# kokutoupan/burn_raymarching

Hardware: AMD Instinct MI355X
Metric: Mrays/s fwd+bwd, 512x512 / 256 spheres / 32 steps, at 1/2/4/8 MI355X (higher is better)
Workload: dtype f32

## Files before the change

burn_raymarching_amd/csrc/rm_kernels.hip:

```cpp
#include <hip/hip_runtime.h>
#include <hip/hip_ext.h>

#include <algorithm>
#include <cstdarg>
#include <cmath>
#include <cstdio>
#include <cstdlib>
#include <cstring>
#include <string>
#include <type_traits>
#include <utility>
#include <vector>

#include "../../include/raymarch.h"
#include "rm_device.h"

namespace rm {

constexpr int kOrderClasses = 16;
constexpr int kOrderClsStride = 32;
constexpr int kOrderCntStride = kOrderClasses * kOrderClsStride > 64 ? kOrderClasses * kOrderClsStride : 64;
static_assert(kOrderCntStride >= kOrderClasses * kOrderClsStride && kOrderCntStride % 32 == 0, "128-byte lines per set");
constexpr int kRedArrStride = 32;

// ... 688 lines not shown
    const int w = __builtin_amdgcn_readfirstlane(*a.oturn);
    const int r = (w + 2) % 3, z = (w + 1) % 3;
    constexpr long long kSet = (long long)kOrderClasses * kMaxBlocksPerLaunch;
    if (o.list_r != nullptr) {
      o.list_r += r * kSet;
      o.cnt_r += r * kOrderCntStride;
    }
    if (o.list_w != nullptr) {
      o.list_w += w * kSet;
      o.cnt_w += w * kOrderCntStride;
    }
    if (o.cnt_z != nullptr) o.cnt_z += z * kOrderCntStride;
  }
  return o;
}

__device__ __forceinline__ long long ray_block(const KArgs& a) {
  int b = blockIdx.x;
  if (a.block_order == nullptr) return b;
  const int g = b >> 3;
  if ((g + 1) * 8 <= (int)gridDim.x) b = (g << 3) + (((b & 7) + g) & 7);
  const OrderSets os = order_sets(a);
  if (os.cnt_r != nullptr) {
    int tot = 0, cb = -1, base = 0;
#pragma unroll
    for (int c = 0; c < kOrderClasses; ++c) {
      const int n = os.cnt_r[c * kOrderClsStride];
      if (cb < 0 && b < tot + n) {
        cb = c;
        base = tot;
      }
      tot += n;
    }
    if (tot == (int)gridDim.x && cb >= 0) return os.list_r[cb * kMaxBlocksPerLaunch + (b - base)];
  }
  const int r = b / a.order_views, v = b - r * a.order_views;
  return (long long)v * a.order_tiles + a.block_order[r];
}

__device__ __forceinline__ void order_append(const KArgs& a, long long blk, int cost) {
  constexpr int kCls = kOrderClasses;
  const float cls_scale = (float)kCls / (float)((a.split ? 1 : kWaves) * (a.steps + kPostCost) + 1);
  const int c = kCls - 1 - (int)fminf((float)cost * cls_scale, (float)(kCls - 1));
  const OrderSets os = order_sets(a);
  const int idx = atomicAdd(os.cnt_w + c * kOrderClsStride, 1);
  if (idx < kMaxBlocksPerLaunch) os.list_w[c * kMaxBlocksPerLaunch + idx] = (int)blk;
}

__device__ __forceinline__ float progress_of(const KArgs& a) {
  if (a.sdev == nullptr) return a.progress;
  return fminf((float)a.sdev->index / (float)a.sdev->total, 1.0f);
}

template <int MODE>
__device__ __forceinline__ void escaped_block(const KArgs& a, const Lds& L, long long blk, long long ri, bool valid,
                                           int tid, int lane, int wave) {
  if (MODE != kBwd && a.out != nullptr && valid) {
    a.out[3 * ri] = 0.0f;
    a.out[3 * ri + 1] = 0.0f;
    a.out[3 * ri + 2] = 0.0f;
  }
  if constexpr (MODE == kFwd || MODE == kRender) return;
  float* rec = a.partials + blk * a.rec;
  float loss = 0.0f;
  if (MODE == kTrain && valid) {
    const float t0 = a.targets[3 * ri], t1 = a.targets[3 * ri + 1], t2 = a.targets[3 * ri + 2];
    const float W = (t0 + t1 + t2) > 0.01f ? 10.0f : fmaf(progress_of(a), 4.0f, 1.0f);
    const float tg[3] = {t0, t1, t2};
#pragma unroll
    for (int c = 0; c < 3; ++c) loss = fmaf(fabsf(0.0f - tg[c]), W, loss);
  }
  const float vals[8] = {0.0f, 0.0f, 0.0f, 0.0f, loss, 0.0f, 0.0f, 0.0f};
  const float red = wave_reduce8(vals, lane);
  if ((lane & 7) == 7) L.slots[wave * 8 + (lane >> 3)] = red;
  __syncthreads();
  if (tid < 8) {
    float acc = L.slots[tid];
#pragma unroll
    for (int w = 1; w < kWaves; ++w) acc += L.slots[w * 8 + tid];
    rec[(long long)a.Mpad * 8 + tid] = acc;
  }
}

template <bool CAM>
__device__ __forceinline__ void setup_ray(const KArgs& a, long long& ri, float o[3], float d[3], int& view) {
  view = 0;
  if constexpr (CAM) {
    const long long npix = (long long)a.width * a.height;
    const int v = (int)(ri / npix);
    view = v;
    const long long pix = ri - (long long)v * npix;
    int x, y;
    if (a.tiling == 2) {
      const long long tl = pix >> 8;
      const int w = (int)(pix & 255), tiles_x = a.width >> 4;
      const int ty = (int)(tl / tiles_x), tx = (int)(tl - (long long)ty * tiles_x);
      const int qd = w >> 6, l = w & 63;
      y = (ty << 4) + ((qd >> 1) << 3) + (l >> 3);
      x = (tx << 4) + ((qd & 1) << 3) + (l & 7);
    } else {
      y = (int)(pix / a.width);
      x = (int)(pix - (long long)y * a.width);
    }
    ri = (long long)v * npix + (long long)y * a.width + x;
    if (a.cams_dev != nullptr) camera_ray(a.cams_dev[v], x, y, a.width, a.height, o, d);
    else camera_ray(a.cams[v], x, y, a.width, a.height, o, d);
  } else {
    o[0] = a.org[3 * ri];
    o[1] = a.org[3 * ri + 1];
    o[2] = a.org[3 * ri + 2];
    d[0] = a.dir[3 * ri];
    d[1] = a.dir[3 * ri + 1];
    d[2] = a.dir[3 * ri + 2];
  }
}

template <int MODE, bool CAM>
__global__ __launch_bounds__(kBlock) void rm_escape_kernel(const KArgs a, int* __restrict__ flags) {
  __shared__ float scratch[8 * kWaves];
  const int tid = threadIdx.x;
  const long long blk = ray_block(a);
  const long long li = blk * kBlock + tid;
  const bool valid = li < a.n_rays;
  long long ri = a.ray_begin + (valid ? li : 0);
  float o[3], d[3];
  int view;
  setup_ray<CAM>(a, ri, o, d, view);
  float c0[3], R;
  scene_bound(a, scratch, tid, c0, R);
  const bool have_t = MODE == kBwd && a.t_in != nullptr;
  const bool esc = !valid || escapes(o, d, have_t ? a.t_in[ri] : -1.0f, have_t, a.steps, c0, R, a.lse_slack,
                                     a.cull_min_d);
  const int all = __syncthreads_and(esc);
  if (tid == 0) flags[blk] = all;
}

#include "rm_ray.h"
#include "rm_reduce.h"
#include "rm_small.h"
#include "rm_raygrad.h"
#include "rm_view.h"
#include "rm_sdf.h"
#include "rm_sh.h"

__global__ __launch_bounds__(64) void rm_stall_kernel(const int* flag, unsigned long long max_ticks) {
  const unsigned long long t0 = __builtin_amdgcn_s_memrealtime();
  while (__hip_atomic_load(flag, __ATOMIC_RELAXED, __HIP_MEMORY_SCOPE_SYSTEM) == 0) {
    if (__builtin_amdgcn_s_memrealtime() - t0 > max_ticks) break;
    __builtin_amdgcn_s_sleep(100);
  }
}

}

#include "rm_context.h"
#include "rm_launch.h"
#include "rm_api.h"
```

burn_raymarching_amd/csrc/rm_proof.h:

```cpp
#pragma once

constexpr int kProofMinSpheres = 128;
constexpr int kLatticeN = 64;
constexpr float kLatticeMargin = 0.25f;
constexpr float kProofMinStep = 0.02f;

constexpr double kMarchAbs = 1e-3;
constexpr double kBoundStepAbs = 1e-3;
constexpr double kRadiusRel = 1e-6;
constexpr double kEscapeRel = 1e-5;
constexpr double kProofRel = 2e-5;
constexpr double kProofMaxMagnitude = 256.0;
constexpr double kLatticeHalfDiag = 0.8660254;
constexpr double kLatticeCellRel = 1e-4;
constexpr double kLatticeKernelAbs = 1e-3;
constexpr double kTileRootRel = 1e-6;
constexpr double kTileRootFloor = 1e-15;
constexpr double kTileLatticeRel = 2e-6;
constexpr double kTileRoundAbs = 1e-4;
constexpr double kTileConeRel = 1e-4;
constexpr double kTileConeAbs = 2e-6;
constexpr double kTileRecedeRel = 2e-6;
constexpr double kBallAbs = kMarchAbs + kBoundStepAbs;
constexpr double kTileLatticeAbs = kMarchAbs + kBoundStepAbs + kLatticeKernelAbs + kTileRoundAbs;
constexpr double kProofDistUp = 1.0000200005;
static_assert(kProofDistUp * (1.0 - kProofRel) >= 1.0 && kProofDistUp < 1.0 + 1.01 * kProofRel,
              "T kProofDistUp >= T / (1 - kProofRel), and no more than it has to be");
static_assert(kLatticeHalfDiag * (1.0 + kLatticeCellRel) > 0.86602540379 * (1.0 + 4e-5),
              "the slack's factor covers sqrt(3)/2 and the cell index's (1/2 + 2e-5) h per axis");
static_assert(kProofRel >= 2.0 * kEscapeRel && kTileLatticeAbs >= kBallAbs + kLatticeKernelAbs,
              "the bound point's test holds the march's own; the tile's lattice term charges what the cell's does");

__device__ __forceinline__ float proof_rprime(float R, float lse_slack) {
  return (R + lse_slack + (float)kMarchAbs) * (1.0f + (float)kRadiusRel);
}
```

burn_raymarching_amd/csrc/rm_ray.h:

```cpp
#pragma once

struct ContState {
  enum Row { kT = 0, kLb, kDprev, kCycT1, kCycT2, kCode, kRhoLb, kRhist, kRayRows };
  static constexpr int kGroupWords = 2;
  struct Ray {
    float t, lb, Dprev, cyc_t1, cyc_t2, rho_lb;
    int rhist;
    bool gone, retired;
  };
  float* cs;
  long long R;
  __host__ __device__ static size_t floats(long long rays, long long groups) {
    return (size_t)(kRayRows * rays + kGroupWords * groups);
  }
  __device__ __forceinline__ explicit ContState(const KArgs& a) : cs(a.cont_state), R(a.cont_rays) {}
  __device__ __forceinline__ float& row(int r, long long li) const { return cs[r * R + li]; }
  __device__ __forceinline__ float& group(long long blk, int w) const { return cs[kRayRows * R + kGroupWords * blk + w]; }
  __device__ __forceinline__ static float code(const Ray& s) { return s.gone ? 1.0f : (s.retired ? 2.0f : 0.0f); }
  __device__ __forceinline__ Ray load(long long li) const {
    Ray s;
    s.t = row(kT, li);
    s.lb = row(kLb, li);
    s.Dprev = row(kDprev, li);
    s.cyc_t1 = row(kCycT1, li);
// ... 49 lines not shown
      const float4 C3 = R4[lay.pair(RecLayout::kP3, i)];
      const float2 C4 = R2[i];
      s.rr = h ? R.w : R.z;
      s.cr = h ? C3.y : C3.x;
      s.cg = h ? C3.w : C3.z;
      s.cbl = h ? C4.y : C4.x;
    } else {
      s.kr = h ? R.y : R.x;
    }
  }
  return s;
}
__device__ __forceinline__ void add_cols4(float* rec, int j, const float (&v)[8]) {
  float4* dst = reinterpret_cast<float4*>(rec + (long long)j * 8);
  float4 o = dst[0];
  o.x += v[0];
  o.y += v[1];
  o.z += v[2];
  o.w += v[3];
  dst[0] = o;
}

template <int MODE, bool CAM, bool SPLIT, bool PROOF>
__device__ __forceinline__ void ray_body(const KArgs& a);

template <int MODE, bool CAM, bool SPLIT, bool PROOF>
__device__ __forceinline__ void ray_entry(const KArgs& a) {
#ifdef RM_BLOCK_TRACE
  const unsigned long long t_begin = __builtin_amdgcn_s_memrealtime();
  ray_body<MODE, CAM, SPLIT, PROOF>(a);
  const unsigned long long t_end = __builtin_amdgcn_s_memrealtime();
  if (a.btrace != nullptr && (threadIdx.x & 63) == 0) {
    const unsigned hw = __builtin_amdgcn_s_getreg((31 << 11) | 4);
    const unsigned xcc = __builtin_amdgcn_s_getreg((31 << 11) | 20);
    unsigned long long* r = a.btrace + kTraceWords * ((unsigned long long)blockIdx.x * kWaves + (threadIdx.x >> 6));
    r[0] = t_begin;
    r[1] = t_end;
    r[2] = (unsigned long long)hw | ((unsigned long long)xcc << 32);
    r[3] = (unsigned long long)ray_block(a) | ((unsigned long long)blockIdx.x << 32);
  }
#else
  ray_body<MODE, CAM, SPLIT, PROOF>(a);
#endif
}
template <int MODE, bool CAM, bool SPLIT, bool PROOF = false>
__global__ __launch_bounds__(kBlock, SPLIT ? kSplitMinWaves : kMinWavesPerSimd) void rm_ray_kernel(const KArgs a) {
  static_assert(!PROOF || (!SPLIT && MODE != kRender), "the escape proof: unsplit training kernels");
  ray_entry<MODE, CAM, SPLIT, PROOF>(a);
}

template <int MODE, bool CAM, bool SPLIT, bool PROOF>
__device__ __forceinline__ void ray_body(const KArgs& a) {
  extern __shared__ __attribute__((aligned(16))) unsigned char smem[];
  const Lds L = bind_lds(a, smem);

  const int tid = threadIdx.x, lane = tid & 63, wave = __builtin_amdgcn_readfirstlane(tid >> 6);
  long long blk;
  long long li_listed = -1;
  bool listed = true;
  if (SPLIT && a.cont_resume > 0 && a.ray_cont) {
    const int n = *a.ray_count;
    const int i0 = (int)blockIdx.x * kSplitRays;
    if (i0 >= n) return;
    const int i = i0 + (lane & (kSplitRays - 1));
    listed = i < n;
    li_listed = a.ray_list[listed ? i : i0];
    blk = -1;
  } else if (SPLIT && a.cont_resume > 0) {
    if ((int)blockIdx.x >= *a.cont_count) return;
    blk = a.cont_list[blockIdx.x];
  } else {
    blk = ray_block(a);
  }
  const long long li = li_listed >= 0 ? li_listed
                                      : (SPLIT ? blk * kSplitRays + (lane & (kSplitRays - 1)) : blk * kBlock + tid);
  const bool valid = listed && li < a.n_rays;
  long long ri = a.ray_begin + (valid ? li : 0);
  const bool own_rays = !SPLIT || (wave == 0 && lane < kSplitRays);

  const float kappa = a.k * kLog2e, nkappa = -kappa, inv_kappa = 1.0f / kappa;

  float o[3], d[3];
  int view;
  setup_ray<CAM>(a, ri, o, d, view);

  if (a.ocnt_z != nullptr && blockIdx.x == 0 && tid < kOrderClasses) order_sets(a).cnt_z[tid * kOrderClsStride] = 0;
  if (a.esc_flags != nullptr && blk >= 0 && a.esc_flags[blk]) {
    if (a.stats != nullptr && tid == 0) atomicAdd(a.stats, 1ull);
    if (a.ocnt_w != nullptr && tid == 0) order_append(a, blk, 0);
    escaped_block<MODE>(a, L, blk, ri, valid, tid, lane, wave);
    return;
  }

  const cf1_ptr hdr = rec_header(L, a.Mpad);
  const float rmin = hdr[Hdr::kRmin], rmax = hdr[Hdr::kRmax], spread = hdr[Hdr::kSpread];
  const bool shift_fixed_ok = !a.shift_max && kappa * (rmax + spread) * 1.001f <= 100.0f;
  const bool shift_none_ok = !a.shift_max && kappa * rmax * 1.001f <= 30.0f;
  const float kr_first = kappa * a.radius[0];
  bool gone = false;
  bool retired = false;
  float rho_lb = -INFINITY;
  const float onorm = fabsf(o[0]) + fabsf(o[1]) + fabsf(o[2]);
  auto rho_moved = [&](float rl, float t0, float t1) {
    return rl - (fabsf(t1 - t0) * 1.000001f + 1e-6f * (1.0f + onorm + fmaxf(t0, t1)));
  };
  auto all_safe = [&](float dist_lb, float rlb) {
    return __all(dist_lb + rmin >= kSafeRho || rlb >= kSafeRho || gone) != 0;
  };
  int split_par = 0;

  auto soft_min = [&](const float p[3], bool fast, float& m, float& s) {
    m = -INFINITY;
    s = 0.0f;
    if (fast)
      lse_point<false, kShiftMax>(p, L, a.Mpad / 2, nkappa, m, s);
    else
      lse_point<true, kShiftMax>(p, L, a.Mpad / 2, nkappa, m, s);
    return -(flog2(fmaxf(s, 1e-8f)) + m) * inv_kappa;
  };
  auto split_pair = [&](int w) { return (((a.Mpad / 2) * w) / kSplitWaves) & ~7; };
  auto soft_min_split = [&](const float p[3], bool fast, float& m, float& s) {
    const int b0 = split_pair(wave), b1 = split_pair(wave + 1);
    const Lds Lq = L.from_pair(b0);
    m = -INFINITY;
    s = 0.0f;
    if (fast) lse_point<false, kShiftMax>(p, Lq, b1 - b0, nkappa, m, s);
    else lse_point<true, kShiftMax>(p, Lq, b1 - b0, nkappa, m, s);
    float* xm = L.slots;
    float* xs = L.slots + kSplitWaves * 64;
    __syncthreads();
    xm[wave * 64 + lane] = m;
    xs[wave * 64 + lane] = s;
    __syncthreads();
    float mm = xm[lane];
#pragma unroll
    for (int w = 1; w < kSplitWaves; ++w) mm = fmaxf(mm, xm[w * 64 + lane]);
    float ss = 0.0f;
#pragma unroll
    for (int w = 0; w < kSplitWaves; ++w) ss += xs[w * 64 + lane] * fexp2(xm[w * 64 + lane] - mm);
    m = mm;
    s = ss;
    return -(flog2(fmaxf(s, 1e-8f)) + m) * inv_kappa;
  };
  auto shade_merge = [&](float c10l, float& dmin, f2& Zw, f2 (&C)[3], f2& Zb, f2 (&G)[3]) {
    constexpr int kF = 9;
    float* xb = L.slots + 2 * kSplitWaves * 64;
    const float v[kF] = {dmin, Zw.x + Zw.y, C[0].x + C[0].y, C[1].x + C[1].y, C[2].x + C[2].y,
                         Zb.x + Zb.y, G[0].x + G[0].y, G[1].x + G[1].y, G[2].x + G[2].y};
#pragma unroll
    for (int f = 0; f < kF; ++f) xb[(f * kSplitWaves + wave) * 64 + lane] = v[f];
    __syncthreads();
    float dm = xb[lane];
#pragma unroll
    for (int w = 1; w < kSplitWaves; ++w) dm = fminf(dm, xb[w * 64 + lane]);
    float acc[kF - 1] = {0.0f, 0.0f, 0.0f, 0.0f, 0.0f, 0.0f, 0.0f, 0.0f};
#pragma unroll
    for (int w = 0; w < kSplitWaves; ++w) {
      const float dw = xb[w * 64 + lane];
      const float sw = fexp2((dm - dw) * c10l), sb = fexp2((dm - dw) * kappa);
#pragma unroll
      for (int f = 1; f < kF; ++f) acc[f - 1] = fmaf(xb[(f * kSplitWaves + w) * 64 + lane], f < 5 ? sw : sb, acc[f - 1]);
    }
    dmin = dm;
    Zw = f2{acc[0], 0.0f};
    C[0] = f2{acc[1], 0.0f};
    C[1] = f2{acc[2], 0.0f};
    C[2] = f2{acc[3], 0.0f};
    Zb = f2{acc[4], 0.0f};
    G[0] = f2{acc[5], 0.0f};
    G[1] = f2{acc[6], 0.0f};
    G[2] = f2{acc[7], 0.0f};
  };
#ifdef RM_BLOCK_TRACE
  unsigned long long tr_paths = 0, tr_lse_cyc = 0, tr_vec = 0;
// ... 155 lines not shown
          lat_inv_h = lg[Lat::kInvH];
          lat_slack = lg[Lat::kSlack] + (float)kBallAbs;
        }
      }
      float u = t;
      bool proven = gone || !valid;
      for (int n = st; n < a.steps; ++n) {
        const float ex = fmaf(d[0], u, o[0]) - c0x, ey = fmaf(d[1], u, o[1]) - c0y, ez = fmaf(d[2], u, o[2]) - c0z;
        const float dist = fsqrt(fmaf(ez, ez, fmaf(ey, ey, ex * ex)));
        const float Tn = esc_tab[min(a.steps - n, kEscTab - 1)];
        proven = proven || (fmaf(ez, d[2], fmaf(ey, d[1], ex * d[0])) >= 0.0f && dist * (1.0f - (float)kProofRel) >= Tn);
        if (__all(proven)) {
          steps_saved += a.steps - st;
          return true;
        }
        float Lb = dist - rs;
        if constexpr (CAM) {
          if (lat) {
            constexpr float kN = (float)kLatticeN;
            const int ix = (int)__builtin_floorf(__builtin_amdgcn_fmed3f((ex + lat_half) * lat_inv_h, -1.0f, kN));
            const int iy = (int)__builtin_floorf(__builtin_amdgcn_fmed3f((ey + lat_half) * lat_inv_h, -1.0f, kN));
            const int iz = (int)__builtin_floorf(__builtin_amdgcn_fmed3f((ez + lat_half) * lat_inv_h, -1.0f, kN));
            const bool inside = (unsigned)(ix | iy | iz) < (unsigned)kLatticeN;
            const int cx = min(max(ix, 0), kLatticeN - 1), cy = min(max(iy, 0), kLatticeN - 1),
                      cz = min(max(iz, 0), kLatticeN - 1);
            const float g = a.lattice[(cz * kLatticeN + cy) * kLatticeN + cx];
            Lb = fmaxf(Lb, inside ? g - lat_slack : -INFINITY);
          }
        }
        if (__any(!proven && !(Lb > kProofMinStep))) return false;
        u += proven ? 0.0f : Lb;
      }
      return false;
    };
    int st_stop = -1;
    int st0 = 0;
#ifdef RM_BLOCK_TRACE
    const unsigned long long tr_c_begin = __builtin_readcyclecounter();
    unsigned long long tr_cyc = 0;
#endif
    if constexpr (CAM) {
      if (a.origin != nullptr && a.steps > 0 && !(SPLIT && a.cont_resume > 0)) {
        const float D0 = a.origin[RecTail::kD0 + view];
        rho_lb = a.origin[RecTail::kRhoLb + view];
        if (__all((__float_as_uint(D0) & 0x7fffffffu) <= 0x7f800000u)) {
          const float p[3] = {fmaf(d[0], t, o[0]), fmaf(d[1], t, o[1]), fmaf(d[2], t, o[2])};
          if (wave_escaped(0, p)) {
            dead = true;
          } else {
            t = fminf(t + (gone ? gone_step : D0), kTMax);
            rho_lb = rho_moved(rho_lb, 0.0f, t);
            lb = D0 - fabsf(D0);
            Dprev = D0;
            st0 = 1;
            steps_saved = 1;
          }
        }
      }
    }
    float cyc_t1 = __builtin_nanf(""), cyc_t2 = __builtin_nanf("");
    int chist = 0xFFF;
    float Dprev2 = INFINITY;
    int rhist = 0xFFF;
    if (SPLIT && a.cont_resume > 0) {
      const ContState cs(a);
      const ContState::Ray s = cs.load(li);
      t = s.t;
      lb = s.lb;
      Dprev = s.Dprev;
      cyc_t1 = s.cyc_t1;
      cyc_t2 = s.cyc_t2;
      gone = s.gone;
      retired = s.retired;
      rho_lb = s.rho_lb;
      rhist = s.rhist;
      if (!a.ray_cont) {
        chist = __float_as_int(cs.group(blk, 0));
        steps_saved = __float_as_int(cs.group(blk, 1));
      }
      st0 = a.cont_resume;
    }
    if constexpr (PROOF) {
      bool taken = false;
      if constexpr (CAM) {
        if (!dead && a.tile_proof != nullptr) taken = a.tile_proof[blk * kWaves + wave] != 0;
      }
      if (taken) {
        steps_saved += a.steps - st0;
        dead = true;
      } else if (!dead && bound_proof(st0)) {
        dead = true;
      }
    }
    const unsigned long long below = (1ull << lane) - 1ull;
    for (int st = st0; !dead && st < a.steps; ++st) {
      if (SPLIT && a.cont_cap > 0 && st == a.cont_cap) {
        const ContState cs(a);
        const bool act = valid && !gone && !retired && lane < kSplitRays;
        gone_finish(st);
        if (wave == 0 && lane < kSplitRays && valid)
          cs.save(li, ContState::Ray{t, lb, Dprev, cyc_t1, cyc_t2, rho_lb, rhist, gone, retired});
        if (wave == 0) {
          const unsigned long long am = __ballot(act);
          const int na = __popcll(am);
          int base = 0;
          if (lane == 0 && na > 0) base = atomicAdd(a.ray_count_w, na);
          base = __shfl(base, 0);
          if (act) a.ray_list_w[base + __popcll(am & below)] = (int)li;
          if (lane == 0) {
            if (!a.ray_cont) {
              cs.group(blk, 0) = __int_as_float(chist);
              cs.group(blk, 1) = __int_as_float(steps_saved + (a.steps - st));
              a.cont_list_w[atomicAdd(a.cont_count_w, 1)] = (int)blk;
            } else if (a.stats != nullptr && st > st0) {
              atomicAdd(a.stats + 2, (unsigned long long)(-(long long)(st - st0)));
            }
          }
        }
        return;
      }
      const float p[3] = {fmaf(d[0], t, o[0]), fmaf(d[1], t, o[1]), fmaf(d[2], t, o[2])};
      if (wave_escaped(st, p)) {
        dead = true;
        st_stop = st;
        break;
      }
      int choice;
      const Memo mm{t, cyc_t1, cyc_t2, Dprev2, chist};
      const float D = soft_min_march(p, all_safe(lb, rho_lb), Dprev, choice, mm);
      const float t_step = t;
      if constexpr (SPLIT) {
        const float rl0 = rho_lb;
        if (!retired) {
          t = fminf(t + (gone ? gone_step : D), kTMax);
          rho_lb = rho_moved(rl0, t_step, t);
          lb = D - fabsf(D);
          Dprev = D;
        }
        if (a.early_exit && MODE != kRender) {
          if (!retired && !gone && valid && t_step == cyc_t2 && (choice & 3) == ((rhist >> 3) & 3)) {
            retired = true;
            if (((a.steps - st) & 1) == 0) {
              t = t_step;
              rho_lb = rl0;
            }
          }
          if (!retired) {
            cyc_t2 = cyc_t1;
            cyc_t1 = t_step;
          }
          rhist = ((rhist << 3) | choice) & 0xFFF;
          if (__all(gone || !valid || retired)) {
            if (gone) gone_steps(st + 1);
            steps_saved += a.steps - 1 - st;
            break;
          }
        }
        continue;
      }
      t = fminf(t + (gone ? gone_step : D), kTMax);
      rho_lb = rho_moved(rho_lb, t_step, t);
      lb = D - fabsf(D);
      Dprev2 = Dprev;
      Dprev = D;
      if (a.early_exit && MODE != kRender) {
        if (choice == ((chist >> 3) & 7) && __all(gone || t_step == cyc_t2)) {
          constexpr int P = 2;
// ... 122 lines not shown
    if constexpr (MODE == kRender) {
      ldn[0] = a.light_fixed[0];
      ldn[1] = a.light_fixed[1];
      ldn[2] = a.light_fixed[2];
    } else {
      amb = a.ambient[0];
      light_unit(a.light_dir, ldn);
    }
    sdot = fmaf(nrm[2], ldn[2], fmaf(nrm[1], ldn[1], nrm[0] * ldn[0]));
    dif = fmaxf(sdot, 0.0f);
    Lgt = MODE == kRender ? dif + 0.1f : fmaf(dif, 1.0f - amb, amb);

    Zw = Zw2.x + Zw2.y;
    Zb = Zb2.x + Zb2.y;
    Df = dmin - flog2(fmaxf(Zb, 1e-8f)) * inv_kappa;
    if constexpr (MODE == kRender) {
      const float e = fexp2(-c10l * dmin);
      const float den = Zw * e + 1e-5f;
      mix[0] = (C2[0].x + C2[0].y) * e / den;
      mix[1] = (C2[1].x + C2[1].y) * e / den;
      mix[2] = (C2[2].x + C2[2].y) * e / den;
      mu = fexp2(-10.0f * kLog2e * Df * Df);
    } else {
      const float invZw0 = frcp(Zw);
      mix[0] = (C2[0].x + C2[0].y) * invZw0;
      mix[1] = (C2[1].x + C2[1].y) * invZw0;
      mix[2] = (C2[2].x + C2[2].y) * invZw0;
      mu = frcp(1.0f + fexp2(a.msharp * kLog2e * Df));
    }
  }
  const float invZw = frcp(Zw);
  const float scale = Lgt * mu;
  const float outv[3] = {mix[0] * scale, mix[1] * scale, mix[2] * scale};

  if (MODE == kFwd && a.dbg != nullptr && valid && own_rays) {
    float* q = a.dbg + 24 * ri;
    const float vals[24] = {t, tf, nrm[0], nrm[1], nrm[2], Lgt, mix[0], mix[1], mix[2], Df, mu, sdot, dmin,
                            Zw, Zb, 0.0f, D6[0], D6[1], D6[2], D6[3], D6[4], D6[5], 0.0f, 0.0f};
#pragma unroll
    for (int c = 0; c < 24; ++c) q[c] = vals[c];
  }
  const bool write_out = MODE != kBwd && a.out != nullptr && valid && own_rays;
  if (write_out) {
    a.out[3 * ri] = outv[0];
    a.out[3 * ri + 1] = outv[1];
    a.out[3 * ri + 2] = outv[2];
  }
  RM_TRACE(5, __builtin_amdgcn_s_memrealtime());
  if constexpr (MODE == kFwd || MODE == kRender) return;

  float g[3] = {0.0f, 0.0f, 0.0f};
  float loss = 0.0f;
  if (valid && own_rays) {
    if constexpr (MODE == kBwd) {
      g[0] = a.gout[3 * ri];
      g[1] = a.gout[3 * ri + 1];
      g[2] = a.gout[3 * ri + 2];
    } else {
      const float t0 = a.targets[3 * ri], t1 = a.targets[3 * ri + 1], t2 = a.targets[3 * ri + 2];
      const float W = (t0 + t1 + t2) > 0.01f ? 10.0f : fmaf(progress_of(a), 4.0f, 1.0f);
      const float tg[3] = {t0, t1, t2};
#pragma unroll
      for (int c = 0; c < 3; ++c) {
        const float df = outv[c] - tg[c];
        loss = fmaf(fabsf(df), W, loss);
        const float sg = df > 0.0f ? 1.0f : (df < 0.0f ? -1.0f : 0.0f);
        g[c] = W * sg * a.inv_count;
      }
    }
  }

  const float gdotm = fmaf(g[2], mix[2], fmaf(g[1], mix[1], g[0] * mix[0]));
  const float gm[3] = {g[0] * scale, g[1] * scale, g[2] * scale};
  const float gL = gdotm * mu, gmu = gdotm * Lgt;
  const float gamb = gL * (1.0f - dif);
  const float gs = sdot >= 0.0f ? gL * (1.0f - amb) : 0.0f;
  const float gell[3] = {gs * nrm[0], gs * nrm[1], gs * nrm[2]};
  const float cmu = gmu * mu * (1.0f - mu) * (-a.msharp);
  const float mg = fmaf(mix[2], gm[2], fmaf(mix[1], gm[1], mix[0] * gm[0]));
  const float b_scale = cmu * frcp(Zb);

  float* rec = a.partials + blk * a.rec;

  static_assert(2 * kWaves <= 8, "misc layout: flags before the scalars");
  int* wflag = reinterpret_cast<int*>(L.misc);
  float* wscal = L.misc + 8;
  {
    const float vals[8] = {gell[0], gell[1], gell[2], gamb, loss, 0.0f, 0.0f, 0.0f};
    const float red = wave_reduce8(vals, lane);
    if ((lane & 7) == 7) wscal[wave * 8 + (lane >> 3)] = red;
    if (lane == 0) {
      wflag[wave] = dead ? 1 : 0;
      wflag[kWaves + wave] = steps_saved;
    }
  }
  auto handoff_work = [&]() {
    if (a.ocnt_w != nullptr) {
      int cost = 0;
#pragma unroll
      for (int w = 0; w < (SPLIT ? 1 : kWaves); ++w) cost += a.steps - wflag[kWaves + w] + (wflag[w] ? 0 : kPostCost);
      order_append(a, blk, cost);
    }
    if (a.stats != nullptr) {
      int ex = 0, sv = 0;
#pragma unroll
      for (int w = 0; w < (SPLIT ? 1 : kWaves); ++w) {
        ex += wflag[w];
        sv += wflag[kWaves + w];
      }
      if (ex != 0) atomicAdd(a.stats + 1, (unsigned long long)ex);
      if (sv != 0) atomicAdd(a.stats + 2, (unsigned long long)sv);
    }
  };
  auto escaped_record = [&]() {
    if (lane < 8) {
      float acc = wscal[lane];
#pragma unroll
      for (int w = 1; w < (SPLIT ? kSplitWaves : kWaves); ++w) acc += wscal[w * 8 + lane];
      rec[(long long)a.Mpad * 8 + lane] = acc;
    }
  };
  __syncthreads();
  int alive = 0;
#pragma unroll
  for (int w = 0; w < (SPLIT ? kSplitWaves : kWaves); ++w) alive |= wflag[w] ? 0 : (1 << w);
  alive = __builtin_amdgcn_readfirstlane(alive);
  if (lane == 0 && wave == (alive != 0 ? __builtin_ctz(alive) : 0)) handoff_work();
  if (dead) {
    if (alive == 0 && wave == 0) escaped_record();
    return;
  }
  const int arank = __popc(alive & ((1 << wave) - 1));

  bool any_seed = true;
  {
    constexpr int kFields = kBwdFields;
    constexpr int kWv = SPLIT ? kSplitWaves : kWaves;
    float* rayf_all = L.slots;
    float* rayf = rayf_all + wave * 64 * kFields;
    float* gta = L.slots + kWaves * 64 * kFields;
    int* nsrc = reinterpret_cast<int*>(L.misc) + 40;
    const RecLayout lay(a.Mpad);
    const float4* R4 = reinterpret_cast<const float4*>(a.rec_buf);
    const float2* R2 = reinterpret_cast<const float2*>(R4 + lay.p4_first());
    const int ngrp = (a.Mpad + 63) / 64;
    auto pair = [&](int sw, int f, int s) {
      return *reinterpret_cast<const f2*>(rayf_all + (sw * kFields + f) * 64 + s);
    };
    const unsigned long long below = (1ull << lane) - 1ull;
    auto unit_range = [&](int r, int nsw, int ncw, int& u0, int& u1) {
      const int U = ngrp * nsw;
      u0 = (r * U) / ncw;
      u1 = ((r + 1) * U) / ncw;
    };
    auto sources = [&]() {
      int m = 0;
#pragma unroll
      for (int sw = 0; sw < kWv; ++sw)
        if ((alive >> sw) & 1) m |= nsrc[sw] > 0 ? (1 << sw) : 0;
      return __builtin_amdgcn_readfirstlane(m);
    };
    auto has_split = [&](int nsw, int ncw) {
      const int U = ngrp * nsw;
      for (int r = 1; r < ncw; ++r)
        if (((r * U) / ncw) % nsw != 0) return true;
      return false;
    };
    auto finish_split = [&](int nsw, int ncw, int crank, bool in, int ncomp, const float (&p0)[8],
                            const float (&p1)[8]) __attribute__((always_inline)) {
      __syncthreads();
      const int nst = ncomp == 8 ? 7 : 4;
      float* mine = rayf_all + crank * 64 * kFields;
      if (in) {
#pragma unroll
        for (int c = 0; c < 7; ++c)
          if (c < nst) {
            mine[c * 64 + lane] = p0[c];
            mine[(nst + c) * 64 + lane] = p1[c];
          }
      }
      __syncthreads();
      if (!in) return;
      int u0, u1;
      unit_range(crank, nsw, ncw, u0, u1);
      if (u1 <= u0) return;
      const int gl = (u1 - 1) / nsw;
      const int kb = max(u0, gl * nsw) - gl * nsw;
      if (kb != 0 || u1 - gl * nsw >= nsw) return;
      float acc[8];
      const int own_slot = (u0 / nsw == gl) ? 0 : 1;
#pragma unroll
      for (int c = 0; c < 8; ++c) acc[c] = c < nst ? mine[(nst * own_slot + c) * 64 + lane] : 0.0f;
      for (int rr = crank + 1; rr < ncw; ++rr) {
        int v0, v1;
        unit_range(rr, nsw, ncw, v0, v1);
        if (v0 >= (gl + 1) * nsw) break;
        if (v1 <= v0) continue;
        const float* part = rayf_all + rr * 64 * kFields;
#pragma unroll
        for (int c = 0; c < 7; ++c)
          if (c < nst) acc[c] += part[c * 64 + lane];
      }
      const int j = gl * 64 + lane;
      if (ncomp == 8) {
        store_group_cols(rec + (long long)gl * 64 * 8, acc, lane, min(64, a.Mpad - gl * 64));
      } else if (j < a.Mpad) {
        add_cols4(rec, j, acc);
      }
    };

    const unsigned long long act1 = __ballot(gm[0] != 0.0f || gm[1] != 0.0f || gm[2] != 0.0f || b_scale != 0.0f);
    const int n1 = __popcll(act1), rank1 = __popcll(act1 & below);
    const bool on1 = ((act1 >> lane) & 1ull) != 0ull;
// ... 220 lines not shown
```

Baseline: 2395.

## Retire tile-proven waves early in training and backward kernels before ray setup

For camera, non-split proof kernels in train/bwd modes, each wave now reads its tile-proof byte before building the ray and, if proven, writes zero output, computes only loss/gradient scalars, publishes its handoff flags and exits. Partially proven blocks let the remaining waves perform the barrier and handoff, with an 'anchor' wave chosen to write the escaped record. This avoids camera ray generation, header loads and the march loop for proven waves, and lets those waves leave before the block barrier. In exchange it adds a more intricate barrier protocol in which not every wave reaches __syncthreads, which is a correctness risk.

```diff
diff --git a/burn_raymarching_amd/csrc/rm_kernels.hip b/burn_raymarching_amd/csrc/rm_kernels.hip
--- a/burn_raymarching_amd/csrc/rm_kernels.hip
+++ b/burn_raymarching_amd/csrc/rm_kernels.hip
@@ -794,29 +794,113 @@
   }
 }
 
+static_assert(2 * kWaves <= 8, "misc layout: flags before the scalars");
+__device__ __forceinline__ int* handoff_flags(const Lds& L) { return reinterpret_cast<int*>(L.misc); }
+__device__ __forceinline__ float* handoff_scalars(const Lds& L) { return L.misc + 8; }
+
+template <int MODE>
+__device__ __forceinline__ void proven_wave(const KArgs& a, const Lds& L, long long blk, long long ri, bool valid,
+                                         int lane, int wave, bool all) {
+  static_assert(MODE == kTrain || MODE == kBwd, "the escape proof: training kernels");
+  if (MODE != kBwd && a.out != nullptr && valid) {
+    a.out[3 * ri] = 0.0f;
+    a.out[3 * ri + 1] = 0.0f;
+    a.out[3 * ri + 2] = 0.0f;
+  }
+  float g[3] = {0.0f, 0.0f, 0.0f};
+  float loss = 0.0f;
+  if (valid) {
+    if constexpr (MODE == kBwd) {
+      g[0] = a.gout[3 * ri];
+      g[1] = a.gout[3 * ri + 1];
+      g[2] = a.gout[3 * ri + 2];
+    } else {
+      const float t0 = a.targets[3 * ri], t1 = a.targets[3 * ri + 1], t2 = a.targets[3 * ri + 2];
+      const float W = (t0 + t1 + t2) > 0.01f ? 10.0f : fmaf(progress_of(a), 4.0f, 1.0f);
+      const float tg[3] = {t0, t1, t2};
+#pragma unroll
+      for (int c = 0; c < 3; ++c) {
+        const float df = 0.0f - tg[c];
+        loss = fmaf(fabsf(df), W, loss);
+        const float sg = df > 0.0f ? 1.0f : (df < 0.0f ? -1.0f : 0.0f);
+        g[c] = W * sg * a.inv_count;
+      }
+    }
+  }
+  const float zero = 0.0f;
+  const float gdotm = fmaf(g[2], zero, fmaf(g[1], zero, g[0] * zero));
+  const float gL = gdotm * zero;
+  const float gamb = gL * (1.0f - zero);
+  const float gs = gL * (1.0f - zero);
+  const float gell = gs * zero;
+  const float vals[8] = {gell, gell, gell, gamb, loss, 0.0f, 0.0f, 0.0f};
+  const float red = wave_reduce8(vals, lane);
+  int* wflag = handoff_flags(L);
+  float* wscal = handoff_scalars(L);
+  if ((lane & 7) == 7) wscal[wave * 8 + (lane >> 3)] = red;
+  if (lane == 0) {
+    wflag[wave] = 1;
+    wflag[kWaves + wave] = a.steps;
+  }
+#ifdef RM_BLOCK_TRACE
+  {
+    const unsigned long long now = __builtin_amdgcn_s_memrealtime();
+    RM_TRACE(4, now);
+    RM_TRACE(5, now);
+    RM_TRACE(6, (unsigned long long)a.steps);
+    for (int w = 7; w < kTraceWords; ++w) RM_TRACE(w, 0ull);
+  }
+#endif
+  if (!all) {
+    __builtin_amdgcn_fence(__ATOMIC_RELEASE, "workgroup");
+    return;
+  }
+  __syncthreads();
+  if (wave != 0) return;
+  if (lane < 8) {
+    float acc = wscal[lane];
+#pragma unroll
+    for (int w = 1; w < kWaves; ++w) acc += wscal[w * 8 + lane];
+    a.partials[blk * a.rec + (long long)a.Mpad * 8 + lane] = acc;
+  }
+  if (lane == 0) {
+    if (a.ocnt_w != nullptr) order_append(a, blk, 0);
+    if (a.stats != nullptr) {
+      atomicAdd(a.stats + 1, (unsigned long long)kWaves);
+      if (a.steps != 0) atomicAdd(a.stats + 2, (unsigned long long)(kWaves * a.steps));
+    }
+  }
+}
+
+__device__ __forceinline__ void camera_pixel(const KArgs& a, long long& ri, int& v, int& x, int& y) {
+  const long long npix = (long long)a.width * a.height;
+  v = (int)(ri / npix);
+  const long long pix = ri - (long long)v * npix;
+  if (a.tiling == 2) {
+    const long long tl = pix >> 8;
+    const int w = (int)(pix & 255), tiles_x = a.width >> 4;
+    const int ty = (int)(tl / tiles_x), tx = (int)(tl - (long long)ty * tiles_x);
+    const int qd = w >> 6, l = w & 63;
+    y = (ty << 4) + ((qd >> 1) << 3) + (l >> 3);
+    x = (tx << 4) + ((qd & 1) << 3) + (l & 7);
+  } else {
+    y = (int)(pix / a.width);
+    x = (int)(pix - (long long)y * a.width);
+  }
+  ri = (long long)v * npix + (long long)y * a.width + x;
+}
+__device__ __forceinline__ void pixel_ray(const KArgs& a, int v, int x, int y, float o[3], float d[3]) {
+  if (a.cams_dev != nullptr) camera_ray(a.cams_dev[v], x, y, a.width, a.height, o, d);
+  else camera_ray(a.cams[v], x, y, a.width, a.height, o, d);
+}
 template <bool CAM>
 __device__ __forceinline__ void setup_ray(const KArgs& a, long long& ri, float o[3], float d[3], int& view) {
   view = 0;
   if constexpr (CAM) {
-    const long long npix = (long long)a.width * a.height;
-    const int v = (int)(ri / npix);
+    int v, x, y;
+    camera_pixel(a, ri, v, x, y);
     view = v;
-    const long long pix = ri - (long long)v * npix;
-    int x, y;
-    if (a.tiling == 2) {
-      const long long tl = pix >> 8;
-      const int w = (int)(pix & 255), tiles_x = a.width >> 4;
-      const int ty = (int)(tl / tiles_x), tx = (int)(tl - (long long)ty * tiles_x);
-      const int qd = w >> 6, l = w & 63;
-      y = (ty << 4) + ((qd >> 1) << 3) + (l >> 3);
-      x = (tx << 4) + ((qd & 1) << 3) + (l & 7);
-    } else {
-      y = (int)(pix / a.width);
-      x = (int)(pix - (long long)y * a.width);
-    }
-    ri = (long long)v * npix + (long long)y * a.width + x;
-    if (a.cams_dev != nullptr) camera_ray(a.cams_dev[v], x, y, a.width, a.height, o, d);
-    else camera_ray(a.cams[v], x, y, a.width, a.height, o, d);
+    pixel_ray(a, v, x, y, o, d);
   } else {
     o[0] = a.org[3 * ri];
     o[1] = a.org[3 * ri + 1];
diff --git a/burn_raymarching_amd/csrc/rm_proof.h b/burn_raymarching_amd/csrc/rm_proof.h
--- a/burn_raymarching_amd/csrc/rm_proof.h
+++ b/burn_raymarching_amd/csrc/rm_proof.h
@@ -31,6 +31,32 @@
 static_assert(kProofRel >= 2.0 * kEscapeRel && kTileLatticeAbs >= kBallAbs + kLatticeKernelAbs,
               "the bound point's test holds the march's own; the tile's lattice term charges what the cell's does");
 
+constexpr int proof_mask(unsigned word) {
+  return ((word & 0xffu) != 0 ? 1 : 0) | ((word & 0xff00u) != 0 ? 2 : 0) | ((word & 0xff0000u) != 0 ? 4 : 0) |
+         ((word & 0xff000000u) != 0 ? 8 : 0);
+}
+constexpr bool proof_all(int mask) { return mask == 15; }
+constexpr int proof_anchor(int mask) {
+  return (mask & 1) == 0 ? 0 : ((mask & 2) == 0 ? 1 : ((mask & 4) == 0 ? 2 : ((mask & 8) == 0 ? 3 : 0)));
+}
+static_assert(proof_mask(0u) == 0 && proof_mask(0x01010101u) == 15 && proof_mask(0x00000001u) == 1 &&
+                  proof_mask(0x00000100u) == 2 && proof_mask(0x00010000u) == 4 && proof_mask(0x01000000u) == 8 &&
+                  proof_mask(0x01000100u) == 10 && proof_mask(0xff000002u) == 9,
+              "byte w of the word is wave w's");
+static_assert(proof_anchor(0) == 0 && proof_anchor(1) == 1 && proof_anchor(2) == 0 && proof_anchor(3) == 2 &&
+                  proof_anchor(4) == 0 && proof_anchor(5) == 1 && proof_anchor(6) == 0 && proof_anchor(7) == 3 &&
+                  proof_anchor(8) == 0 && proof_anchor(9) == 1 && proof_anchor(10) == 0 && proof_anchor(11) == 2 &&
+                  proof_anchor(12) == 0 && proof_anchor(13) == 1 && proof_anchor(14) == 0 && proof_anchor(15) == 0,
+              "the anchor of each of the 16 masks: its lowest clear bit");
+static_assert(!proof_all(0) && !proof_all(1) && !proof_all(2) && !proof_all(3) && !proof_all(4) && !proof_all(5) &&
+                  !proof_all(6) && !proof_all(7) && !proof_all(8) && !proof_all(9) && !proof_all(10) && !proof_all(11) &&
+                  !proof_all(12) && !proof_all(13) && !proof_all(14) && proof_all(15),
+              "all proven: mask 15 alone");
+static_assert(((1 >> proof_anchor(1)) & 1) == 0 && ((3 >> proof_anchor(3)) & 1) == 0 && ((5 >> proof_anchor(5)) & 1) == 0 &&
+                  ((7 >> proof_anchor(7)) & 1) == 0 && ((9 >> proof_anchor(9)) & 1) == 0 && ((11 >> proof_anchor(11)) & 1) == 0 &&
+                  ((13 >> proof_anchor(13)) & 1) == 0 && ((14 >> proof_anchor(14)) & 1) == 0,
+              "an anchor's own byte is 0: it reaches the barrier");
+
 __device__ __forceinline__ float proof_rprime(float R, float lse_slack) {
   return (R + lse_slack + (float)kMarchAbs) * (1.0f + (float)kRadiusRel);
 }
diff --git a/burn_raymarching_amd/csrc/rm_ray.h b/burn_raymarching_amd/csrc/rm_ray.h
--- a/burn_raymarching_amd/csrc/rm_ray.h
+++ b/burn_raymarching_amd/csrc/rm_ray.h
@@ -155,7 +155,10 @@
 
   float o[3], d[3];
   int view;
-  setup_ray<CAM>(a, ri, o, d, view);
+  constexpr bool kLeave = PROOF && CAM && !SPLIT && (MODE == kTrain || MODE == kBwd);
+  int px = 0, py = 0;
+  if constexpr (kLeave) camera_pixel(a, ri, view, px, py);
+  else setup_ray<CAM>(a, ri, o, d, view);
 
   if (a.ocnt_z != nullptr && blockIdx.x == 0 && tid < kOrderClasses) order_sets(a).cnt_z[tid * kOrderClsStride] = 0;
   if (a.esc_flags != nullptr && blk >= 0 && a.esc_flags[blk]) {
@@ -163,6 +166,17 @@
     if (a.ocnt_w != nullptr && tid == 0) order_append(a, blk, 0);
     escaped_block<MODE>(a, L, blk, ri, valid, tid, lane, wave);
     return;
+  }
+  if constexpr (kLeave) {
+    static_assert(kWaves == 4, "proof_mask: four bytes, one word");
+    if (a.tile_proof != nullptr && (MODE != kBwd || a.t_in == nullptr)) {
+      const int pmask = proof_mask(*reinterpret_cast<const unsigned*>(a.tile_proof + blk * kWaves));
+      if ((pmask >> wave) & 1) {
+        proven_wave<MODE>(a, L, blk, ri, valid, lane, wave, proof_all(pmask));
+        return;
+      }
+    }
+    pixel_ray(a, view, px, py, o, d);
   }
 
   const cf1_ptr hdr = rec_header(L, a.Mpad);
@@ -484,7 +498,7 @@
     }
     if constexpr (PROOF) {
       bool taken = false;
-      if constexpr (CAM) {
+      if constexpr (CAM && MODE == kFwd) {
         if (!dead && a.tile_proof != nullptr) taken = a.tile_proof[blk * kWaves + wave] != 0;
       }
       if (taken) {
@@ -773,7 +787,6 @@
 
   float* rec = a.partials + blk * a.rec;
 
-  static_assert(2 * kWaves <= 8, "misc layout: flags before the scalars");
   int* wflag = reinterpret_cast<int*>(L.misc);
   float* wscal = L.misc + 8;
   {
@@ -816,10 +829,21 @@
 #pragma unroll
   for (int w = 0; w < (SPLIT ? kSplitWaves : kWaves); ++w) alive |= wflag[w] ? 0 : (1 << w);
   alive = __builtin_amdgcn_readfirstlane(alive);
-  if (lane == 0 && wave == (alive != 0 ? __builtin_ctz(alive) : 0)) handoff_work();
-  if (dead) {
-    if (alive == 0 && wave == 0) escaped_record();
-    return;
+  if constexpr (kLeave) {
+    int anchor = 0;
+    if (alive == 0 && a.tile_proof != nullptr && (MODE != kBwd || a.t_in == nullptr))
+      anchor = proof_anchor(proof_mask(*reinterpret_cast<const unsigned*>(a.tile_proof + blk * kWaves)));
+    if (lane == 0 && wave == (alive != 0 ? __builtin_ctz(alive) : anchor)) handoff_work();
+    if (dead) {
+      if (alive == 0 && wave == anchor) escaped_record();
+      return;
+    }
+  } else {
+    if (lane == 0 && wave == (alive != 0 ? __builtin_ctz(alive) : 0)) handoff_work();
+    if (dead) {
+      if (alive == 0 && wave == 0) escaped_record();
+      return;
+    }
   }
   const int arank = __popc(alive & ((1 << wave) - 1));
 
```

Result: no change. 2412 (median of 4 runs) (+0.7%).
